# Sandy4321/dist-svgd

Hardware: AMD Instinct MI355X
Metric: SVGD particle-updates/sec (n=65536,d=256) at 1/2/4/8 GPUs + % MFMA/HBM roofline (higher is better)
Workload: dtype f32; 1 GPU; dist-logreg DistSampler all_scores, Jacobi, median bandwidth; n=65536, d=256, N_global=16384, parallelism=dp1, particles_per_gpu=65536

## Files before the change

### dist-svgd_amd/csrc/gemm_x3.hpp

```cpp
#pragma once
#include "gemm_tiles.hpp"

namespace dsvgd {

typedef __bf16 bf16x8 __attribute__((ext_vector_type(8)));
typedef __bf16 bf16x4 __attribute__((ext_vector_type(4)));
typedef uint32_t u32x4 __attribute__((ext_vector_type(4)));
typedef uint32_t u32x2 __attribute__((ext_vector_type(2)));

__device__ __forceinline__ f32x16 mfma_bf16(bf16x8 a, bf16x8 b, f32x16 c) {
  return __builtin_amdgcn_mfma_f32_32x32x16_bf16(a, b, c, 0, 0, 0);
}

struct Split3 {
  __bf16 s0, s1, s2;
};
__device__ __forceinline__ Split3 split3(float v) {
  Split3 o;
  o.s0 = (__bf16)v;
  float r = v - (float)o.s0;
  o.s1 = (__bf16)r;
  r -= (float)o.s1;
  o.s2 = (__bf16)r;
  return o;
}

constexpr int kX3Parts = 3;
constexpr int kX3Step = 16;

__device__ __forceinline__ float lane_select(uint64_t mask, float a, float b) {
  float d;
  asm("v_cndmask_b32 %0, %1, %2, %3" : "=v"(d) : "v"(b), "v"(a), "s"(mask));
  return d;
}

typedef _Float16 f16x8 __attribute__((ext_vector_type(8)));
typedef _Float16 f16x4 __attribute__((ext_vector_type(4)));

struct FmtX3 {
  using E = __bf16;
  using V8 = bf16x8;
  using V4 = bf16x4;
  static constexpr int P = 3;
  static constexpr float kAScale = 1.f;
  static constexpr float kAScaleLog2 = 0.f;
};
struct FmtH2 {
  using E = _Float16;
  using V8 = f16x8;
  using V4 = f16x4;
  static constexpr int P = 2;
  static constexpr float kAScale = 32768.f;
  static constexpr float kAScaleLog2 = 15.f;
};

template <class F>
__device__ __forceinline__ f32x16 mfma_fmt(typename F::V8 a, typename F::V8 b, f32x16 c) {
  if constexpr (F::P == 3)
    return __builtin_amdgcn_mfma_f32_32x32x16_bf16(a, b, c, 0, 0, 0);
  else
    return __builtin_amdgcn_mfma_f32_32x32x16_f16(a, b, c, 0, 0, 0);
}

template <class F>
__device__ __forceinline__ void split_fmt(float v, typename F::E (&o)[F::P]) {
  if constexpr (F::P == 3) {
    const Split3 s = split3(v);
    o[0] = s.s0;
    o[1] = s.s1;
    o[2] = s.s2;
  } else {
    o[0] = (_Float16)v;
    o[1] = (_Float16)(v - (float)o[0]);
  }
}

template <class F, int TM>
__device__ __forceinline__ void mfma_products(const typename F::V8 (&a)[TM][F::P],
                                              const typename F::V8 (&b)[F::P], f32x16* acc) {
  if constexpr (F::P == 3) {
#pragma unroll
    for (int mi = 0; mi < TM; ++mi) acc[mi] = mfma_fmt<F>(a[mi][2], b[0], acc[mi]);
#pragma unroll
    for (int mi = 0; mi < TM; ++mi) acc[mi] = mfma_fmt<F>(a[mi][1], b[1], acc[mi]);
#pragma unroll
    for (int mi = 0; mi < TM; ++mi) acc[mi] = mfma_fmt<F>(a[mi][0], b[2], acc[mi]);
  }
#pragma unroll
  for (int mi = 0; mi < TM; ++mi) acc[mi] = mfma_fmt<F>(a[mi][1], b[0], acc[mi]);
#pragma unroll
  for (int mi = 0; mi < TM; ++mi) acc[mi] = mfma_fmt<F>(a[mi][0], b[1], acc[mi]);
#pragma unroll
  for (int mi = 0; mi < TM; ++mi) acc[mi] = mfma_fmt<F>(a[mi][0], b[0], acc[mi]);
}

__device__ __forceinline__ int x3_off(int x, int h) { return x * 32 + ((h ^ ((x >> 3) & 1)) << 4); }

template <int TN, bool DMA = true, bool EXP = true, bool M16 = false, int RW = 2, class F = FmtX3,
          int NB = 2, int FAM = kFamRBF>
struct NNX3Tile {
  static constexpr int P = F::P;
  static_assert(NB == 2 || (NB == 3 && DMA), "3-stage ring: DMA path");
  static constexpr int ND = NB;
  using V8 = typename F::V8;
  static_assert(!M16 || P == 3, "the 16x16x32 concatenated-k form is the 3-part format's");
  static constexpr int kThreads = 512;
  static constexpr int TM = 2;
  static constexpr int kCW = 8 / RW;
  static constexpr int BM = 64 * RW;
  static constexpr int AR = BM / 128;
  static constexpr int BC = kCW * 32 * TN;
  static_assert(RW == 2 || (RW == 4 && DMA && !EXP), "256-row blocks: DMA path, no exp");
  static constexpr int BJ = kX3Step;
  static constexpr int SA = P * BM * 32;
  static constexpr int SB = P * BC * 32;
  static constexpr int kStage = SA + SB;
  static constexpr int kSmemBytes = NB * kStage + (DMA ? ND * AR * kPanelElems * 4 : 0);
  static constexpr int kBChunks = SB / 16;
  static constexpr int LB = (kBChunks + kThreads - 1) / kThreads;
  static constexpr int kHalf = TN > 1 ? TN / 2 : 1;
  static_assert(kSmemBytes <= 160 * 1024, "LDS budget");
  static_assert(!DMA || kBChunks % kThreads == 0, "DMA: every wave issues LB DMAs");

  f32x16 acc[TM][TN];
  f32x4 acc16[4][2 * TN];
  bf16x8 a16[4][3];
  f32x4 ra;
  int64_t prow = 0;
  u32x4 rb[DMA ? 1 : LB];
  float rs;
  float pw;
  V8 a[TM][P];

  __device__ __forceinline__ float kval(float v, float scale) const {
    if constexpr (FAM == kFamIMQ)
      return imq_pow(v, scale, pw, F::kAScaleLog2);
    else
      return __builtin_amdgcn_exp2f(fmaf(v, scale, F::kAScaleLog2));
  }

  __device__ __forceinline__ void load(const float* __restrict__ Apanels, const typename F::E* __restrict__ Yx,
                                       int64_t ldy, int64_t j0) {
    const int t = threadIdx.x;
    const __amdgpu_buffer_rsrc_t rA =
        __builtin_amdgcn_make_buffer_rsrc((void*)Apanels, (short)0, 0x7fffffff, 0x00020000);
    const __amdgpu_buffer_rsrc_t rB =
        __builtin_amdgcn_make_buffer_rsrc((void*)Yx, (short)0, 0x7fffffff, 0x00020000);
    const int soA = (int)((j0 >> 4) * kPanelElems * 4);
    const int soB = (int)((j0 >> 4) * P * ldy * 32);
    ra = __builtin_bit_cast(f32x4, __builtin_amdgcn_raw_buffer_load_b128(rA, t * 16, soA, 0));
#pragma unroll
    for (int u = 0; u < LB; ++u) {
      const int f = t + u * kThreads;
      if (kBChunks % kThreads == 0 || f < kBChunks) {
        const int p = f / (2 * BC), rem = f % (2 * BC);
        rb[u] = __builtin_bit_cast(
            u32x4, __builtin_amdgcn_raw_buffer_load_b128(rB, (int)(p * ldy * 32 + rem * 16), soB, 0));
      }
    }
  }

  __device__ __forceinline__ void store(char* st, float scale, int64_t dgl) {
    store_a(st, scale, dgl);
    const int t = threadIdx.x;
#pragma unroll
    for (int u = 0; u < LB; ++u) {
      const int f = t + u * kThreads;
      if (kBChunks % kThreads == 0 || f < kBChunks)
        *reinterpret_cast<u32x4*>(st + SA + f * 16) = rb[u];
    }
  }

  __device__ __forceinline__ void store_a(char* st, float scale, int64_t dgl, int a = 0) {
    const int t = threadIdx.x, row = (t >> 2) + 128 * a, c4 = t & 3;
    if (!EXP) {
      if constexpr (F::kAScale != 1.f) {
#pragma unroll
        for (int q = 0; q < 4; ++q) ra[q] *= F::kAScale;
      }
    } else if (dgl > -BM && dgl < BJ) {
      const int qd = (int)dgl + row - 4 * c4;
#pragma unroll
      for (int q = 0; q < 4; ++q)
        ra[q] = (qd == q) ? 0.f : kval(ra[q], scale);
    } else {
#pragma unroll
      for (int q = 0; q < 4; ++q) ra[q] = kval(ra[q], scale);
    }
    if (EXP) rs += (ra[0] + ra[1]) + (ra[2] + ra[3]);
    typename F::V4 sp[P];
#pragma unroll
    for (int q = 0; q < 4; ++q) {
      typename F::E v[P];
      split_fmt<F>(ra[q], v);
#pragma unroll
      for (int p = 0; p < P; ++p) sp[p][q] = v[p];
    }
    const int off = (M16 ? row * 32 + ((c4 >> 1) << 4) : x3_off(row, c4 >> 1)) + ((c4 & 1) << 3);
#pragma unroll
    for (int p = 0; p < P; ++p) *reinterpret_cast<typename F::V4*>(st + p * BM * 32 + off) = sp[p];
  }

  static constexpr int kRaw = NB * kStage;
  static constexpr int kSlot = AR * kPanelElems * 4;
  static constexpr int kDAux = 2;

  template <int AUX = 0>
  __device__ __forceinline__ static void dma16(__amdgpu_buffer_rsrc_t r, char* lds, int voff,
                                               int soff) {
    __builtin_amdgcn_raw_ptr_buffer_load_lds(r, (__attribute__((address_space(3))) void*)lds, 16,
                                             voff, soff, 0, AUX);
  }

  __device__ __forceinline__ void dma_b(char* st, __amdgpu_buffer_rsrc_t rB, int64_t ldy,
                                        int64_t j0) {
    const int t = threadIdx.x, wbase = __builtin_amdgcn_readfirstlane(t >> 6) * 64;
    const int soB = (int)((j0 >> 4) * P * ldy * 32);
#pragma unroll
    for (int u = 0; u < LB; ++u) {
      const int f = t + u * kThreads, p = f / (2 * BC), rem = f % (2 * BC);
      dma16(rB, st + SA + (wbase + u * kThreads) * 16, (int)(p * ldy * 32 + rem * 16), soB);
    }
  }

  __device__ __forceinline__ void dma_d(char* raw, __amdgpu_buffer_rsrc_t rA, int64_t j0) {
    const int t = threadIdx.x;
    if (transposed(j0)) {
      const float* src = sym_D + (((j0 >> 7) * sym_pcols + sym_I * 8) * kPanelElems +
                                   (j0 & 127) * 16);
      const __amdgpu_buffer_rsrc_t rT =
          __builtin_amdgcn_make_buffer_rsrc((void*)src, (short)0, 0x7fffffff, 0x00020000);
      dma16<kDAux>(rT, raw + __builtin_amdgcn_readfirstlane(t >> 6) * 1024, (t >> 6) * kPanelElems * 4 + (t & 63) * 16, 0);
      return;
    }
#pragma unroll
    for (int a = 0; a < AR; ++a)
      dma16<kDAux>(rA, raw + a * kPanelElems * 4 + __builtin_amdgcn_readfirstlane(t >> 6) * 1024, (int)(a * prow) + t * 16,
                   (int)((j0 >> 4) * kPanelElems * 4));
  }

  __device__ __forceinline__ f32x4 raw_read(const char* raw, int64_t j0, int a = 0) const {
    const int t = threadIdx.x;
    if (RW == 2 && transposed(j0)) {
      const int row = t >> 2, c4 = t & 3;
      const float* r = reinterpret_cast<const float*>(raw) + (row >> 4) * 256 + (row & 15) +
                       (4 * c4) * 16;
      float v[4];
#pragma unroll
      for (int e = 0; e < 4; ++e) v[e] = r[((e + c4) & 3) * 16];
      constexpr uint64_t kOdd = 0xAAAAAAAAAAAAAAAAull, kHi2 = 0xCCCCCCCCCCCCCCCCull;
      float w[4];
#pragma unroll
      for (int q = 0; q < 4; ++q) w[q] = lane_select(kOdd, v[(q + 3) & 3], v[q]);
#pragma unroll
      for (int q = 0; q < 4; ++q) v[q] = lane_select(kHi2, w[(q + 2) & 3], w[q]);
      return f32x4{v[0], v[1], v[2], v[3]};
    }
    return *reinterpret_cast<const f32x4*>(raw + a * kPanelElems * 4 + t * 16);
  }

  int64_t kst = BJ;
  const float* sym_D = nullptr;
  int64_t sym_pcols = 0;
  int64_t sym_I = 0;
  __device__ __forceinline__ bool transposed(int64_t j0) const {
    return sym_D != nullptr && (j0 >> 7) < sym_I;
  }

  __device__ __forceinline__ void read_a(const char* st, int wr) {
    if (M16) {
      const int lane = threadIdx.x & 63, rr = lane & 15, g = lane >> 4, hh = g & 1;
#pragma unroll
      for (int mt = 0; mt < 4; ++mt) {
        const int off = (wr * 64 + mt * 16 + rr) * 32 + hh * 16;
        const int sl = g >> 1;
        a16[mt][0] = *reinterpret_cast<const bf16x8*>(st + sl * BM * 32 + off);
        a16[mt][1] = *reinterpret_cast<const bf16x8*>(st + (sl ^ 1) * BM * 32 + off);
        a16[mt][2] = *reinterpret_cast<const bf16x8*>(st + 2 * sl * BM * 32 + off);
      }
      return;
    }
    const int lane = threadIdx.x & 63, r = lane & 31, h = lane >> 5;
#pragma unroll
    for (int mi = 0; mi < TM; ++mi)
#pragma unroll
      for (int p = 0; p < P; ++p)
        a[mi][p] = *reinterpret_cast<const V8*>(st + p * BM * 32 +
                                                x3_off(wr * 32 * TM + mi * 32 + r, h));
  }

  template <int N0, int N1>
  __device__ __forceinline__ void compute(const char* st, int wc) {
    if (M16) {
      const int lane = threadIdx.x & 63, rr = lane & 15, g = lane >> 4, hh = g & 1;
      const int s = g >> 1;
#pragma unroll
      for (int nt = 2 * N0; nt < 2 * N1; ++nt) {
        const char* bb = st + SA + (wc * 32 * TN + nt * 16 + rr) * 32 + hh * 16;
        const bf16x8 g1 = *reinterpret_cast<const bf16x8*>(bb + s * BC * 32);
        const bf16x8 g3 = *reinterpret_cast<const bf16x8*>(bb + (2 - 2 * s) * BC * 32);
#pragma unroll
        for (int mt = 0; mt < 4; ++mt)
          acc16[mt][nt] = __builtin_amdgcn_mfma_f32_16x16x32_bf16(a16[mt][2], g3, acc16[mt][nt], 0, 0, 0);
#pragma unroll
        for (int mt = 0; mt < 4; ++mt)
          acc16[mt][nt] = __builtin_amdgcn_mfma_f32_16x16x32_bf16(a16[mt][1], g1, acc16[mt][nt], 0, 0, 0);
#pragma unroll
        for (int mt = 0; mt < 4; ++mt)
          acc16[mt][nt] = __builtin_amdgcn_mfma_f32_16x16x32_bf16(a16[mt][0], g1, acc16[mt][nt], 0, 0, 0);
      }
      return;
    }
    const int lane = threadIdx.x & 63, r = lane & 31, h = lane >> 5;
#pragma unroll
    for (int ni = N0; ni < N1; ++ni) {
      V8 b[P];
#pragma unroll
      for (int p = 0; p < P; ++p)
        b[p] = *reinterpret_cast<const V8*>(st + SA + p * BC * 32 +
                                            x3_off(wc * 32 * TN + ni * 32 + r, h));
      f32x16 c[TM];
#pragma unroll
      for (int mi = 0; mi < TM; ++mi) c[mi] = acc[mi][ni];
      mfma_products<F, TM>(a, b, c);
#pragma unroll
      for (int mi = 0; mi < TM; ++mi) acc[mi][ni] = c[mi];
    }
  }

  __device__ __forceinline__ static void lds_barrier() {
    asm volatile("s_waitcnt lgkmcnt(0)\n\ts_barrier" ::: "memory");
  }

  __device__ __forceinline__ void run(const float* __restrict__ Apanels, const typename F::E* __restrict__ Yx,
                                      int64_t ldy, int64_t k0, int64_t k1, float scale, char* smem,
                                      int64_t row_g0) {
    const int w = __builtin_amdgcn_readfirstlane((int)(threadIdx.x >> 6)), wr = w / kCW, wc = w % kCW;
    rs = 0.f;
#pragma unroll
    for (int mi = 0; mi < TM; ++mi)
#pragma unroll
      for (int ni = 0; ni < TN; ++ni)
#pragma unroll
        for (int q = 0; q < 16; ++q) acc[mi][ni][q] = 0.f;
#pragma unroll
    for (int mt = 0; mt < 4; ++mt)
#pragma unroll
      for (int nt = 0; nt < 2 * TN; ++nt) acc16[mt][nt] = f32x4{0.f, 0.f, 0.f, 0.f};
    if (k0 >= k1) return;
    if (DMA) {
      const __amdgpu_buffer_rsrc_t rA =
          __builtin_amdgcn_make_buffer_rsrc((void*)Apanels, (short)0, 0x7fffffff, 0x00020000);
      const __amdgpu_buffer_rsrc_t rB =
          __builtin_amdgcn_make_buffer_rsrc((void*)Yx, (short)0, 0x7fffffff, 0x00020000);
      char* raw = smem + kRaw;
      if constexpr (NB == 3) {
        dma_b(smem, rB, ldy, k0);
        dma_d(raw, rA, k0);
        if (k0 + kst < k1) {
          dma_b(smem + kStage, rB, ldy, k0 + kst);
          dma_d(raw + kSlot, rA, k0 + kst);
          asm volatile("s_waitcnt vmcnt(%0)" ::"n"(LB + AR) : "memory");
        } else {
          asm volatile("s_waitcnt vmcnt(0)" ::: "memory");
        }
#pragma unroll
        for (int a = 0; a < AR; ++a) {
          ra = raw_read(raw, k0, a);
          store_a(smem, scale, row_g0 - k0, a);
        }
        asm volatile("s_waitcnt lgkmcnt(0)\n\ts_barrier" ::: "memory");
        for (int64_t j0 = k0; j0 < k1; j0 += 3 * kst) {
          step_dma3<0>(rA, rB, ldy, j0, k1, scale, smem, row_g0, wr, wc);
          if (j0 + kst < k1) step_dma3<1>(rA, rB, ldy, j0 + kst, k1, scale, smem, row_g0, wr, wc);
          if (j0 + 2 * kst < k1)
            step_dma3<2>(rA, rB, ldy, j0 + 2 * kst, k1, scale, smem, row_g0, wr, wc);
        }
// ... 318 lines not shown
```

### dist-svgd_amd/csrc/phi_w1.hpp

```cpp
#pragma once
#include "gemm_x3.hpp"

namespace dsvgd {

struct PhiW1 {
  static constexpr int kThreads = 256;
  static constexpr int BM = 128, BC = 512, BJ = 16, P = 2;
  static constexpr int SA = P * BM * 32;
  static constexpr int kSmemBytes = 2 * SA;
  static constexpr int kScrLd = 44;
  static constexpr int kScrBytes = 16 * kScrLd * 4;
};

constexpr int kW1Sgb = 4;
__device__ __forceinline__ f32x4 w1_load(__amdgpu_buffer_rsrc_t r, int voff, int soff) {
  return __builtin_bit_cast(f32x4, __builtin_amdgcn_raw_buffer_load_b128(r, voff, soff, 0));
}
__device__ __forceinline__ f32x4 w1_load_nt(__amdgpu_buffer_rsrc_t r, int voff, int soff) {
  return __builtin_bit_cast(f32x4, __builtin_amdgcn_raw_buffer_load_b128(r, voff, soff, 2));
}

constexpr int w1_waves(int NI, bool EXP) { return NI == 2 && EXP ? 2 : 1; }
template <int DS, int NI = 4, bool EXP = true, int FAM = kFamRBF, class... PW>
__global__ __launch_bounds__(256)
__attribute__((amdgpu_waves_per_eu(w1_waves(NI, EXP), w1_waves(NI, EXP)))) void phi_w1_kernel(
    const float* A, int64_t a_npad, const _Float16* Yx, int64_t ldy,
    int64_t K, int64_t kchunk, const dsvgd_select_state* __restrict__ st, float* __restrict__ C,
    int64_t ldc, float* __restrict__ rowsum, int64_t m, int64_t row0, int sym,
    const float* __restrict__ colinv, int slice0, const float* __restrict__ gate, int gate_on,
    int ks_begin = 0, int ks_wrap = 0, int tcol0 = 0, int t_per = 0, int t_first = 0,
    int t_nblk = 1, int64_t t_ostride = 0, PW... pw_) {
  static_assert(sizeof...(PW) == (FAM == kFamIMQ ? 1 : 0), "pw: the IMQ instantiations only");
  [[maybe_unused]] const float pw = (0.f + ... + pw_);
  static_assert(NI == 4 || NI == 2, "NI: 4 or 2 column tiles per wave");
  static_assert(EXP || DS == 0, "the identity form is DS 0 only");
  const bool want_rs = EXP || rowsum != nullptr;
  if (gate && ((*gate != 0.f) != (gate_on != 0))) return;
  using F = FmtH2;
  constexpr int BC = 4 * 32 * NI;
  using V8 = F::V8;
  constexpr int P = PhiW1::P;
  constexpr bool TRK = DS == 1 || DS == 3 || DS == 4;
  __shared__ __attribute__((aligned(16))) char smem[PhiW1::kSmemBytes + (TRK ? 4 * PhiW1::kScrBytes : 0)];
  const int t = threadIdx.x, lane = t & 63, r = lane & 31, h = lane >> 5;
  const int w = __builtin_amdgcn_readfirstlane(t >> 6);
  const int64_t lin = (int64_t)blockIdx.z * gridDim.y + blockIdx.y;
  const bool xm = ((DS == 4 || DS == 0) && t_per == 1) || (DS == 3 && t_per > 0 && tcol0 == 1);
  const int64_t lid = lin * gridDim.x + blockIdx.x;
  const int64_t xu = (lid >> 3) * (8 / gridDim.z) + (lid & 7) / gridDim.z;
  const int64_t cbx = xm ? xu % gridDim.x : blockIdx.x;
  const int64_t by = xm ? xu / gridDim.x
                   : DS == 2 ? lin / gridDim.z
                   : DS == 1 ? (int64_t)gridDim.y - 1 - lin / gridDim.z : blockIdx.y;
  const int64_t bz = xm ? (lid & 7) % gridDim.z
                   : (DS == 1 || DS == 2) ? lin % gridDim.z : blockIdx.z;
  const bool tb = DS == 3 && t_per > 0;
  const int64_t tpart = tb ? by / t_per : 0;
  const int64_t byl = tb ? by % t_per : by;
  const int64_t i0 = byl * PhiW1::BM;
  const int64_t c0 = cbx * BC + w * 32 * NI;
  const int64_t kb0 = bz * kchunk, kend = min(K, kb0 + kchunk);
  int ks0 = (int)(kb0 / PhiW1::BJ) + (DS == 0 ? ks_begin : 0);
  int nsteps = kend > kb0 ? (int)((kend - kb0) / PhiW1::BJ) : 0;
  const int Z = (int)gridDim.z;
  const int kdir = DS == 2 ? -Z : DS == 1 ? Z : 1;
  auto wrapk = [&](int ks) { return (DS == 0 && ks_wrap > 0 && ks >= ks_wrap) ? ks - ks_wrap : ks; };
  const int kyoff = DS == 3 ? ks_begin : 0;
  if (DS == 2) {
    const int T = (int)((K - i0) / PhiW1::BJ);
    ks0 = (int)(K / PhiW1::BJ) - 1 - (int)bz;
    nsteps = T > bz ? (T - (int)bz + Z - 1) / Z : 0;
  } else if (DS == 1) {
    const int T = (int)(i0 / PhiW1::BJ);
    ks0 = (int)bz;
    nsteps = T > bz ? (T - (int)bz + Z - 1) / Z : 0;
  }
  const int ksp = DS == 4 ? (int)min(max(kb0, i0), kend) / PhiW1::BJ : 0;
  if (tb) {
    const int64_t at = ((int64_t)bz * (gridDim.y / t_per) + tpart) * t_ostride;
    C += at;
    rowsum += at;
  } else {
    C += (int64_t)(slice0 + bz) * m * ldc;
    rowsum += (int64_t)(slice0 + bz) * roundup128(m);
  }
  const float scale = !EXP ? 0.f : FAM == kFamIMQ ? st->inv_h : -st->inv_h * kLog2e;

  const __amdgpu_buffer_rsrc_t rD = __builtin_amdgcn_make_buffer_rsrc(
      (void*)(A + (i0 >> 7) * (a_npad >> 4) * kPanelElems), (short)0, 0x7fffffff, 0x00020000);
  const __amdgpu_buffer_rsrc_t rB =
      __builtin_amdgcn_make_buffer_rsrc((void*)(Yx + c0 * 16), (short)0, 0x7fffffff, 0x00020000);
  const int pstride = (int)(ldy * 32);
  const int vB = x3_off(r, h);
  const int vD = t * 32;
  const int srow = t >> 1, shalf = t & 1;
  const int aoff = x3_off(srow, shalf);
  auto diag0 = [&](int kfirst) {
    int64_t dg = row0 + i0 + srow - 8 * shalf - (int64_t)kfirst * PhiW1::BJ;
    if (DS == 0 && ks_wrap > 0 && row0 + i0 + srow < (int64_t)ks_begin * PhiW1::BJ)
      dg += (int64_t)ks_wrap * PhiW1::BJ;
    return (int)max(min(dg, (int64_t)(1 << 30)), (int64_t)-(1 << 30));
  };

  f32x16 acc[4][NI];
#pragma unroll
  for (int mi = 0; mi < 4; ++mi)
#pragma unroll
    for (int ni = 0; ni < NI; ++ni)
#pragma unroll
      for (int q = 0; q < 16; ++q) acc[mi][ni][q] = 0.f;
  float rs = 0.f;

  const int symI = tb ? (int)(((t_first + tpart) % t_nblk) * t_per + byl)
                   : DS == 3 ? tcol0 + (int)by : (sym || DS == 4) ? (int)(i0 >> 7) : -1;
  const int64_t pcols = a_npad >> 4;
  const int vP = (t >> 5) * kPanelElems * 4 + (t & 31) * 32;
  float* const scr = reinterpret_cast<float*>(smem + PhiW1::kSmemBytes + w * PhiW1::kScrBytes);
  const int sw_off = ((lane & 31) >> 1) * PhiW1::kScrLd + 16 * (lane >> 5) + 8 * (lane & 1);
  const int sr_off = 8 * shalf * PhiW1::kScrLd + (lane >> 1);

  auto phase = [&](auto TR_, const int ks0, const int nsteps, const int qd0) {
    constexpr bool TR = decltype(TR_)::value;
    if (nsteps <= 0) return;
    V8 b[NI][P];
    f32x4 dr[4][2];
    f32x4 tr[2];
    const int last = nsteps - 1;
    auto loadB = [&](int ni, int k) {
      const int soff = (wrapk(ks0 + kdir * min(k, last)) + kyoff) * P * pstride;
#pragma unroll
      for (int p = 0; p < P; ++p)
        b[ni][p] = __builtin_bit_cast(V8, w1_load(rB, vB + ni * 1024, soff + p * pstride));
    };
    auto loadD = [&](f32x4 (&d)[2], int k) {
      const int kc = min(k, last);
      const int64_t j0 = (int64_t)wrapk(ks0 + kdir * kc) * PhiW1::BJ;
      if constexpr (TR) {
        const float* src = A + (((j0 >> 7) * pcols + symI * 8) * kPanelElems + (j0 & 127) * 16);
        const __amdgpu_buffer_rsrc_t rT =
            __builtin_amdgcn_make_buffer_rsrc((void*)src, (short)0, 0x7fffffff, 0x00020000);
        d[0] = w1_load_nt(rT, vP, 0);
        d[1] = w1_load_nt(rT, vP + 16, 0);
      } else {
        const int soff = (int)(j0 >> 4) * kPanelElems * 4;
        d[0] = w1_load_nt(rD, vD, soff);
        d[1] = w1_load_nt(rD, vD + 16, soff);
      }
    };
    auto transpose = [&](const f32x4 (&d)[2], f32x4 (&o)[2]) {
      *reinterpret_cast<f32x4*>(scr + sw_off) = d[0];
      *reinterpret_cast<f32x4*>(scr + sw_off + 4) = d[1];
#pragma unroll
      for (int q = 0; q < 8; ++q) o[q >> 2][q & 3] = scr[sr_off + q * PhiW1::kScrLd];
    };
    auto stage = [&](char* st_, const f32x4 (&d)[2], int k) {
      const int qd = max(min(qd0 - kdir * k * PhiW1::BJ, 8), -1);
      float e[8];
#pragma unroll
      for (int q = 0; q < 8; ++q) {
        const float v = q < 4 ? d[0][q] : d[1][q - 4];
        const float x = !EXP ? v * F::kAScale
                        : FAM == kFamIMQ ? imq_pow(v, scale, pw, F::kAScaleLog2)
                                         : __builtin_amdgcn_exp2f(fmaf(v, scale, F::kAScaleLog2));
        e[q] = (EXP && !TR && qd == q) ? 0.f : x;
      }
      const float s = ((e[0] + e[1]) + (e[2] + e[3])) + ((e[4] + e[5]) + (e[6] + e[7]));
      rs += k <= last ? s : 0.f;
      V8 p0, p1;
#pragma unroll
      for (int q = 0; q < 8; ++q) {
        const _Float16 a0 = (_Float16)e[q];
        p0[q] = a0;
        p1[q] = (_Float16)(e[q] - (float)a0);
      }
      *reinterpret_cast<V8*>(st_ + aoff) = p0;
      *reinterpret_cast<V8*>(st_ + PhiW1::BM * 32 + aoff) = p1;
    };
    auto barrier = []() { asm volatile("s_waitcnt lgkmcnt(0)\n\ts_barrier" ::: "memory"); };
    auto step = [&](int k, const char* cur, char* nxt, const f32x4 (&ds_)[2], f32x4 (&dl)[2],
                    const f32x4 (&dt)[2]) {
      V8 a[4][P];
#pragma unroll
      for (int mi = 0; mi < 4; ++mi)
#pragma unroll
        for (int p = 0; p < P; ++p)
          a[mi][p] = *reinterpret_cast<const V8*>(cur + p * PhiW1::BM * 32 + x3_off(mi * 32 + r, h));
      if constexpr (TR)
        stage(nxt, tr, k + 1);
      else
        stage(nxt, ds_, k + 1);
#pragma unroll
      for (int ni = 0; ni < NI; ++ni) {
#pragma unroll
        for (int mi = 0; mi < 4; ++mi) acc[mi][ni] = mfma_fmt<F>(a[mi][1], b[ni][0], acc[mi][ni]);
#pragma unroll
        for (int mi = 0; mi < 4; ++mi) acc[mi][ni] = mfma_fmt<F>(a[mi][0], b[ni][1], acc[mi][ni]);
#pragma unroll
        for (int mi = 0; mi < 4; ++mi) acc[mi][ni] = mfma_fmt<F>(a[mi][0], b[ni][0], acc[mi][ni]);
        loadB(ni, k + 1);
      }
      if constexpr (TR) transpose(dt, tr);
      __builtin_amdgcn_sched_group_barrier(0x100, 8, 0);
#pragma unroll
      for (int i = 0; i < 4 * NI; ++i) {
        __builtin_amdgcn_sched_group_barrier(0x008, 1, 0);
        __builtin_amdgcn_sched_group_barrier(0x002, kW1Sgb, 0);
      }
      __builtin_amdgcn_sched_group_barrier(0x200, 2, 0);
#pragma unroll
      for (int i = 0; i < 8 * NI; ++i) {
        __builtin_amdgcn_sched_group_barrier(0x008, 1, 0);
        if (TR && i == 1) __builtin_amdgcn_sched_group_barrier(0x200, 2, 0);
        if (TR && i >= 2 && i < 10) __builtin_amdgcn_sched_group_barrier(0x100, 1, 0);
        if (i % 4 == 3) __builtin_amdgcn_sched_group_barrier(0x020, 1, 0);
      }
      loadD(dl, k + 3);
    };

#pragma unroll
    for (int ni = 0; ni < NI; ++ni) loadB(ni, 0);
    loadD(dr[0], 0);
    loadD(dr[1], 1);
    loadD(dr[2], 2);
    if constexpr (TR) {
      transpose(dr[0], tr);
      stage(smem, tr, 0);
      transpose(dr[1], tr);
    } else {
      stage(smem, dr[0], 0);
    }
    barrier();
    for (int k = 0; k < nsteps; k += 8) {
      step(k, smem, smem + PhiW1::SA, dr[1], dr[3], dr[2]);
      barrier();
      if (k + 1 >= nsteps) break;
      step(k + 1, smem + PhiW1::SA, smem, dr[2], dr[0], dr[3]);
      barrier();
      if (k + 2 >= nsteps) break;
      step(k + 2, smem, smem + PhiW1::SA, dr[3], dr[1], dr[0]);
      barrier();
      if (k + 3 >= nsteps) break;
      step(k + 3, smem + PhiW1::SA, smem, dr[0], dr[2], dr[1]);
      barrier();
      if (k + 4 >= nsteps) break;
      step(k + 4, smem, smem + PhiW1::SA, dr[1], dr[3], dr[2]);
      barrier();
      if (k + 5 >= nsteps) break;
      step(k + 5, smem + PhiW1::SA, smem, dr[2], dr[0], dr[3]);
      barrier();
      if (k + 6 >= nsteps) break;
      step(k + 6, smem, smem + PhiW1::SA, dr[3], dr[1], dr[0]);
      barrier();
      if (k + 7 >= nsteps) break;
      step(k + 7, smem + PhiW1::SA, smem, dr[0], dr[2], dr[1]);
      barrier();
    }
  };
  if constexpr (DS == 4) {
    phase(std::true_type{}, ks0, ksp - ks0, 0);
    phase(std::false_type{}, ksp, ks0 + nsteps - ksp, diag0(ksp));
  } else {
    phase(std::integral_constant<bool, DS == 1 || DS == 3>{}, ks0, nsteps, diag0(ks0));
  }

#pragma unroll
  for (int mi = 0; mi < 4; ++mi)
#pragma unroll
    for (int ni = 0; ni < NI; ++ni) {
      const int64_t col = c0 + ni * 32 + r;
      const float cs = colinv[col] * (1.f / F::kAScale);
#pragma unroll
      for (int q = 0; q < 16; ++q) {
        const int64_t row = i0 + mi * 32 + c_row(q, lane);
        if (row < m) C[row * ldc + col] = acc[mi][ni][q] * cs;
      }
    }
  {
    const float v = rs + __shfl_xor(rs, 1, 64);
    if (want_rs && cbx == 0 && shalf == 0 && i0 + srow < m)
      rowsum[i0 + srow] = v * (1.f / F::kAScale);
  }
}

}
```

### dist-svgd_amd/csrc/phi_w2.hpp

```cpp
#pragma once
#include "phi_w1.hpp"

namespace dsvgd {

struct PhiW2 {
  static constexpr int kThreads = 256;
  static constexpr int BM = 256, BC = 256, BJ = 16, P = 2;
  static constexpr int SA = P * BM * 32;
  static constexpr int kSmemBytes = 2 * SA;
};

#ifndef DSVGD_W2_SGB
#define DSVGD_W2_SGB 6
#endif
#ifndef DSVGD_W2_MF
#define DSVGD_W2_MF 40
#endif
constexpr int kW2Sgb = DSVGD_W2_SGB, kW2Mf = DSVGD_W2_MF;

template <int DS>
__global__ __launch_bounds__(256) __attribute__((amdgpu_waves_per_eu(1, 1))) void phi_w2_kernel(
    const float* A, int64_t a_npad, int64_t a_rows, const _Float16* Wh, int64_t ldw, int64_t K,
    int64_t kchunk, const dsvgd_select_state* __restrict__ st, float* __restrict__ C, int64_t ldc,
    float* __restrict__ rowsum, int64_t m, int64_t row0, const float* __restrict__ colinv,
    const float* __restrict__ gate, int xm) {
  static_assert(DS == 0 || DS == 4, "DS: 0 (full layout) or 4 (symmetric, one launch)");
  if (gate && *gate != 0.f) return;
  using F = FmtH2;
  using V8 = F::V8;
  constexpr int P = PhiW2::P, BM = PhiW2::BM;
  constexpr bool SYM = DS == 4;
  __shared__ __attribute__((aligned(16))) char smem[PhiW2::kSmemBytes + (SYM ? 8 * PhiW1::kScrBytes : 0)];
  const int t = threadIdx.x, lane = t & 63, r = lane & 31, h = lane >> 5;
  const int w = __builtin_amdgcn_readfirstlane(t >> 6);
  const int wr = w >> 1, wc = w & 1;
  const int64_t lid = ((int64_t)blockIdx.z * gridDim.y + blockIdx.y) * gridDim.x + blockIdx.x;
  const int64_t xu = (lid >> 3) * (8 / gridDim.z) + (lid & 7) / gridDim.z;
  const int64_t cbx = xm ? xu % gridDim.x : blockIdx.x;
  const int64_t by = xm ? xu / gridDim.x : blockIdx.y;
  const int64_t bz = xm ? (lid & 7) % gridDim.z : blockIdx.z;
  const int64_t i0 = by * BM;
  const int64_t c0 = cbx * PhiW2::BC + wc * 128;
  const int64_t kb0 = bz * kchunk, kend = min(K, kb0 + kchunk);
  const int ks0 = (int)(kb0 / PhiW2::BJ);
  const int nsteps = kend > kb0 ? (int)((kend - kb0) / PhiW2::BJ) : 0;
  C += bz * m * ldc;
  rowsum += bz * roundup128(m);
  const float scale = -st->inv_h * kLog2e;
  const bool live1 = i0 + 128 < a_rows;
  const int64_t pcols = a_npad >> 4;
  const __amdgpu_buffer_rsrc_t rD0 = __builtin_amdgcn_make_buffer_rsrc(
      (void*)(A + (i0 >> 7) * pcols * kPanelElems), (short)0, 0x7fffffff, 0x00020000);
  const __amdgpu_buffer_rsrc_t rD1 = __builtin_amdgcn_make_buffer_rsrc(
      (void*)(A + ((i0 >> 7) + (live1 ? 1 : 0)) * pcols * kPanelElems), (short)0,
      live1 ? 0x7fffffff : 0, 0x00020000);
  const __amdgpu_buffer_rsrc_t rB =
      __builtin_amdgcn_make_buffer_rsrc((void*)(Wh + c0 * 16), (short)0, 0x7fffffff, 0x00020000);
  const int pstride = (int)(ldw * 32);
  const int vB = x3_off(r, h);
  const int vD = t * 32;
  const int srow = t >> 1, shalf = t & 1;
  const int aoff = x3_off(srow, shalf);
  auto diag0 = [&](int kfirst, int hb) {
    const int64_t dg = row0 + i0 + 128 * hb + srow - 8 * shalf - (int64_t)kfirst * PhiW2::BJ;
    return (int)max(min(dg, (int64_t)(1 << 30)), (int64_t)-(1 << 30));
  };

  f32x16 acc[4][4];
#pragma unroll
  for (int mi = 0; mi < 4; ++mi)
#pragma unroll
    for (int ni = 0; ni < 4; ++ni)
#pragma unroll
      for (int q = 0; q < 16; ++q) acc[mi][ni][q] = 0.f;
  float rs0 = 0.f, rs1 = 0.f;

  const int symI = (int)(i0 >> 7);
  const int vP = (t >> 5) * kPanelElems * 4 + (t & 31) * 32;
  float* const scr0 = reinterpret_cast<float*>(smem + PhiW2::kSmemBytes + w * PhiW1::kScrBytes);
  float* const scr1 = scr0 + 4 * (PhiW1::kScrBytes / 4);
  const int sw_off = ((lane & 31) >> 1) * PhiW1::kScrLd + 16 * (lane >> 5) + 8 * (lane & 1);
  const int sr_off = 8 * shalf * PhiW1::kScrLd + (lane >> 1);

  auto phase = [&](auto TR0_, auto TR1_, const int ks0, const int nsteps, const int qd0,
                   const int qd1) {
    constexpr bool TR0 = decltype(TR0_)::value, TR1 = decltype(TR1_)::value;
    if (nsteps <= 0) return;
    V8 b[4][P];
    f32x4 dr[4][2][2];
    f32x4 tr[2][2];
    const int last = nsteps - 1;
    auto loadB = [&](int ni, int k) {
      const int soff = (ks0 + min(k, last)) * P * pstride;
#pragma unroll
      for (int p = 0; p < P; ++p)
        b[ni][p] = __builtin_bit_cast(V8, w1_load(rB, vB + ni * 1024, soff + p * pstride));
    };
    auto loadD = [&](f32x4 (&d)[2][2], int k) {
      const int64_t j0 = (int64_t)(ks0 + min(k, last)) * PhiW2::BJ;
      const int soff = (int)(j0 >> 4) * kPanelElems * 4;
      auto one = [&](auto TR_, int hb, f32x4 (&o)[2]) {
        if constexpr (decltype(TR_)::value) {
          const bool ok = hb == 0 || live1;
          const float* src = A + (((j0 >> 7) * pcols + (symI + (ok ? hb : 0)) * 8) * kPanelElems +
                                  (j0 & 127) * 16);
          const __amdgpu_buffer_rsrc_t rT = __builtin_amdgcn_make_buffer_rsrc(
              (void*)src, (short)0, ok ? 0x7fffffff : 0, 0x00020000);
          o[0] = w1_load_nt(rT, vP, 0);
          o[1] = w1_load_nt(rT, vP + 16, 0);
        } else {
          o[0] = w1_load_nt(hb ? rD1 : rD0, vD, soff);
          o[1] = w1_load_nt(hb ? rD1 : rD0, vD + 16, soff);
        }
      };
      one(TR0_, 0, d[0]);
      one(TR1_, 1, d[1]);
    };
    auto transpose = [&](float* scr, const f32x4 (&d)[2], f32x4 (&o)[2]) {
      *reinterpret_cast<f32x4*>(scr + sw_off) = d[0];
      *reinterpret_cast<f32x4*>(scr + sw_off + 4) = d[1];
#pragma unroll
      for (int q = 0; q < 8; ++q) o[q >> 2][q & 3] = scr[sr_off + q * PhiW1::kScrLd];
    };
    auto stage = [&](char* st_, const f32x4 (&d)[2], int k, bool tr_, int qd0_, float& rs) {
      const int qd = max(min(qd0_ - k * PhiW2::BJ, 8), -1);
      float e[8];
#pragma unroll
      for (int q = 0; q < 8; ++q) {
        const float v = q < 4 ? d[0][q] : d[1][q - 4];
        const float x = __builtin_amdgcn_exp2f(fmaf(v, scale, F::kAScaleLog2));
        e[q] = (!tr_ && qd == q) ? 0.f : x;
      }
      const float s = ((e[0] + e[1]) + (e[2] + e[3])) + ((e[4] + e[5]) + (e[6] + e[7]));
      rs += k <= last ? s : 0.f;
      V8 p0, p1;
#pragma unroll
      for (int q = 0; q < 8; ++q) {
        const _Float16 a0 = (_Float16)e[q];
        p0[q] = a0;
        p1[q] = (_Float16)(e[q] - (float)a0);
      }
      *reinterpret_cast<V8*>(st_ + aoff) = p0;
      *reinterpret_cast<V8*>(st_ + BM * 32 + aoff) = p1;
    };
    auto stage2 = [&](char* st_, const f32x4 (&d)[2][2], int k) {
      if constexpr (TR0) stage(st_, tr[0], k, true, qd0, rs0);
      else stage(st_, d[0], k, false, qd0, rs0);
      if constexpr (TR1) stage(st_ + 128 * 32, tr[1], k, true, qd1, rs1);
      else stage(st_ + 128 * 32, d[1], k, false, qd1, rs1);
    };
    auto barrier = []() { asm volatile("s_waitcnt lgkmcnt(0)\n\ts_barrier" ::: "memory"); };
    auto step = [&](int k, const char* cur, char* nxt, const f32x4 (&ds_)[2][2],
                    f32x4 (&dl)[2][2], const f32x4 (&dt)[2][2]) {
      V8 a[4][P];
#pragma unroll
      for (int mi = 0; mi < 4; ++mi)
#pragma unroll
        for (int p = 0; p < P; ++p)
          a[mi][p] = *reinterpret_cast<const V8*>(cur + p * BM * 32 +
                                                  x3_off(wr * 128 + mi * 32 + r, h));
      stage2(nxt, ds_, k + 1);
#pragma unroll
      for (int ni = 0; ni < 4; ++ni) {
#pragma unroll
        for (int mi = 0; mi < 4; ++mi) acc[mi][ni] = mfma_fmt<F>(a[mi][1], b[ni][0], acc[mi][ni]);
#pragma unroll
        for (int mi = 0; mi < 4; ++mi) acc[mi][ni] = mfma_fmt<F>(a[mi][0], b[ni][1], acc[mi][ni]);
#pragma unroll
        for (int mi = 0; mi < 4; ++mi) acc[mi][ni] = mfma_fmt<F>(a[mi][0], b[ni][0], acc[mi][ni]);
        loadB(ni, k + 1);
      }
      if constexpr (TR0) transpose(scr0, dt[0], tr[0]);
      if constexpr (TR1) transpose(scr1, dt[1], tr[1]);
      __builtin_amdgcn_sched_group_barrier(0x100, 8, 0);
#pragma unroll
      for (int i = 0; i < kW2Mf; ++i) {
        __builtin_amdgcn_sched_group_barrier(0x008, 1, 0);
        __builtin_amdgcn_sched_group_barrier(0x002, kW2Sgb, 0);
        if (i % 12 == 11) __builtin_amdgcn_sched_group_barrier(0x020, 2, 0);
      }
      __builtin_amdgcn_sched_group_barrier(0x200, 4, 0);
#pragma unroll
      for (int i = kW2Mf; i < 48; ++i) {
        __builtin_amdgcn_sched_group_barrier(0x008, 1, 0);
        if (i % 12 == 11) __builtin_amdgcn_sched_group_barrier(0x020, 2, 0);
      }
      loadD(dl, k + 3);
    };

#pragma unroll
    for (int ni = 0; ni < 4; ++ni) loadB(ni, 0);
    loadD(dr[0], 0);
    loadD(dr[1], 1);
    loadD(dr[2], 2);
    if constexpr (TR0) transpose(scr0, dr[0][0], tr[0]);
    if constexpr (TR1) transpose(scr1, dr[0][1], tr[1]);
    stage2(smem, dr[0], 0);
    if constexpr (TR0) transpose(scr0, dr[1][0], tr[0]);
    if constexpr (TR1) transpose(scr1, dr[1][1], tr[1]);
    barrier();
    for (int k = 0; k < nsteps; k += 4) {
      step(k, smem, smem + PhiW2::SA, dr[1], dr[3], dr[2]);
      barrier();
      if (k + 1 >= nsteps) break;
      step(k + 1, smem + PhiW2::SA, smem, dr[2], dr[0], dr[3]);
      barrier();
      if (k + 2 >= nsteps) break;
      step(k + 2, smem, smem + PhiW2::SA, dr[3], dr[1], dr[0]);
      barrier();
      if (k + 3 >= nsteps) break;
      step(k + 3, smem + PhiW2::SA, smem, dr[0], dr[2], dr[1]);
      barrier();
    }
  };
  using T_ = std::true_type;
  using F_ = std::false_type;
  if constexpr (SYM) {
    const int kse = ks0 + nsteps;
    const int ka = min(max(ks0, (int)(i0 >> 4)), kse), kb = min(max(ks0, (int)(i0 >> 4) + 8), kse);
    phase(T_{}, T_{}, ks0, ka - ks0, 0, 0);
    phase(F_{}, T_{}, ka, kb - ka, diag0(ka, 0), 0);
    phase(F_{}, F_{}, kb, kse - kb, diag0(kb, 0), diag0(kb, 1));
  } else {
    phase(F_{}, F_{}, ks0, nsteps, diag0(ks0, 0), diag0(ks0, 1));
  }

#pragma unroll
  for (int mi = 0; mi < 4; ++mi)
#pragma unroll
    for (int ni = 0; ni < 4; ++ni) {
      const int64_t col = c0 + ni * 32 + r;
      const float cs = colinv[col] * (1.f / F::kAScale);
#pragma unroll
      for (int q = 0; q < 16; ++q) {
        const int64_t row = i0 + wr * 128 + mi * 32 + c_row(q, lane);
        if (row < m) C[row * ldc + col] = acc[mi][ni][q] * cs;
      }
    }
  {
    const float v0 = rs0 + __shfl_xor(rs0, 1, 64), v1 = rs1 + __shfl_xor(rs1, 1, 64);
    if (cbx == 0 && shalf == 0) {
      if (i0 + srow < m) rowsum[i0 + srow] = v0 * (1.f / F::kAScale);
      if (i0 + 128 + srow < m) rowsum[i0 + 128 + srow] = v1 * (1.f / F::kAScale);
    }
  }
}

}
```

Before: 4.924 million particle-updates/s.

## Use packed fma_mix f16 split, peel diagonal masking, and retune W1 schedule groups

Replaces the per-element f32→f16 hi/lo split with packed conversions plus v_fma_mixlo/mixhi residual computation in both phi kernels, cutting VALU instructions in the staging path. In phi_w1 the diagonal-zeroing select is peeled out: a wave-uniform ballot checks whether an 8-step block can touch the diagonal and runs a mask-free body otherwise. The row-sum reduction gets asm barriers to fix its association order, and the sched_group_barrier interleave for the NI=2 variant is made tunable and retuned. These changes add inline asm and more code paths, which raises the risk of scheduling or register-pressure regressions.

New measurement: 4.960 million particle-updates/s (median of 6 runs). Within noise of the previous version (+0.7%).

```diff
diff --git a/dist-svgd_amd/csrc/gemm_x3.hpp b/dist-svgd_amd/csrc/gemm_x3.hpp
--- a/dist-svgd_amd/csrc/gemm_x3.hpp
+++ b/dist-svgd_amd/csrc/gemm_x3.hpp
@@ -73,6 +73,28 @@
     o[0] = (_Float16)v;
     o[1] = (_Float16)(v - (float)o[0]);
   }
+}
+
+typedef _Float16 f16x2 __attribute__((ext_vector_type(2)));
+__device__ __forceinline__ void split_h2_pair(float e0, float e1, uint32_t& hi, uint32_t& lo) {
+  const f16x2 h = {(_Float16)e0, (_Float16)e1};
+  hi = __builtin_bit_cast(uint32_t, h);
+  asm("v_fma_mixlo_f16 %0, %1, -1.0, %2 op_sel_hi:[1,0,0]" : "=v"(lo) : "v"(hi), "v"(e0));
+  asm("v_fma_mixhi_f16 %0, %1, -1.0, %2 op_sel:[1,0,0] op_sel_hi:[1,0,0]"
+      : "+v"(lo)
+      : "v"(hi), "v"(e1));
+}
+__device__ __forceinline__ void split_h2_x8(const float (&e)[8], f16x8& p0, f16x8& p1) {
+  u32x4 hi, lo;
+#pragma unroll
+  for (int q = 0; q < 4; ++q) {
+    uint32_t a, b;
+    split_h2_pair(e[2 * q], e[2 * q + 1], a, b);
+    hi[q] = a;
+    lo[q] = b;
+  }
+  p0 = __builtin_bit_cast(f16x8, hi);
+  p1 = __builtin_bit_cast(f16x8, lo);
 }
 
 template <class F, int TM>
diff --git a/dist-svgd_amd/csrc/phi_w1.hpp b/dist-svgd_amd/csrc/phi_w1.hpp
--- a/dist-svgd_amd/csrc/phi_w1.hpp
+++ b/dist-svgd_amd/csrc/phi_w1.hpp
@@ -12,12 +12,43 @@
   static constexpr int kScrBytes = 16 * kScrLd * 4;
 };
 
-constexpr int kW1Sgb = 4;
+#ifndef DSVGD_W1_SGB
+#define DSVGD_W1_SGB 5
+#endif
+#ifndef DSVGD_W1_GAPS
+#define DSVGD_W1_GAPS 8
+#endif
+#ifndef DSVGD_W1_TRANS
+#define DSVGD_W1_TRANS 0
+#endif
+constexpr int w1_sgb(int NI) { return NI == 2 ? DSVGD_W1_SGB : 4; }
+constexpr int w1_gaps(int NI) { return NI == 2 ? DSVGD_W1_GAPS : 4 * NI; }
+constexpr bool w1_sgb_trans(int NI) { return NI == 2 && DSVGD_W1_TRANS != 0; }
+#ifndef DSVGD_W1_SPLIT
+#define DSVGD_W1_SPLIT 1
+#endif
+#ifndef DSVGD_W1_PEEL
+#define DSVGD_W1_PEEL 1
+#endif
+constexpr bool kW1Split = DSVGD_W1_SPLIT != 0, kW1Peel = DSVGD_W1_PEEL != 0;
 __device__ __forceinline__ f32x4 w1_load(__amdgpu_buffer_rsrc_t r, int voff, int soff) {
   return __builtin_bit_cast(f32x4, __builtin_amdgcn_raw_buffer_load_b128(r, voff, soff, 0));
 }
 __device__ __forceinline__ f32x4 w1_load_nt(__amdgpu_buffer_rsrc_t r, int voff, int soff) {
   return __builtin_bit_cast(f32x4, __builtin_amdgcn_raw_buffer_load_b128(r, voff, soff, 2));
+}
+
+__device__ __forceinline__ float w1_sum8(const float (&e)[8]) {
+  float s[4];
+#pragma unroll
+  for (int q = 0; q < 4; ++q) {
+    s[q] = e[2 * q] + e[2 * q + 1];
+    asm("" : "+v"(s[q]));
+  }
+  float a = s[0] + s[1], b = s[2] + s[3];
+  asm("" : "+v"(a));
+  asm("" : "+v"(b));
+  return a + b;
 }
 
 constexpr int w1_waves(int NI, bool EXP) { return NI == 2 && EXP ? 2 : 1; }
@@ -121,6 +152,8 @@
 
   auto phase = [&](auto TR_, const int ks0, const int nsteps, const int qd0) {
     constexpr bool TR = decltype(TR_)::value;
+    constexpr std::true_type yes{};
+    [[maybe_unused]] constexpr std::false_type no{};
     if (nsteps <= 0) return;
     V8 b[NI][P];
     f32x4 dr[4][2];
@@ -153,8 +186,9 @@
 #pragma unroll
       for (int q = 0; q < 8; ++q) o[q >> 2][q & 3] = scr[sr_off + q * PhiW1::kScrLd];
     };
-    auto stage = [&](char* st_, const f32x4 (&d)[2], int k) {
-      const int qd = max(min(qd0 - kdir * k * PhiW1::BJ, 8), -1);
+    auto stage = [&](auto DG_, char* st_, const f32x4 (&d)[2], int k) __attribute__((always_inline)) {
+      constexpr bool DG = decltype(DG_)::value && EXP && !TR;
+      [[maybe_unused]] const int qd = max(min(qd0 - kdir * k * PhiW1::BJ, 8), -1);
       float e[8];
 #pragma unroll
       for (int q = 0; q < 8; ++q) {
@@ -162,23 +196,30 @@
         const float x = !EXP ? v * F::kAScale
                         : FAM == kFamIMQ ? imq_pow(v, scale, pw, F::kAScaleLog2)
                                          : __builtin_amdgcn_exp2f(fmaf(v, scale, F::kAScaleLog2));
-        e[q] = (EXP && !TR && qd == q) ? 0.f : x;
-      }
-      const float s = ((e[0] + e[1]) + (e[2] + e[3])) + ((e[4] + e[5]) + (e[6] + e[7]));
+        if constexpr (DG)
+          e[q] = qd == q ? 0.f : x;
+        else
+          e[q] = x;
+      }
+      const float s = w1_sum8(e);
       rs += k <= last ? s : 0.f;
       V8 p0, p1;
-#pragma unroll
-      for (int q = 0; q < 8; ++q) {
-        const _Float16 a0 = (_Float16)e[q];
-        p0[q] = a0;
-        p1[q] = (_Float16)(e[q] - (float)a0);
+      if constexpr (kW1Split) {
+        split_h2_x8(e, p0, p1);
+      } else {
+#pragma unroll
+        for (int q = 0; q < 8; ++q) {
+          const _Float16 a0 = (_Float16)e[q];
+          p0[q] = a0;
+          p1[q] = (_Float16)(e[q] - (float)a0);
+        }
       }
       *reinterpret_cast<V8*>(st_ + aoff) = p0;
       *reinterpret_cast<V8*>(st_ + PhiW1::BM * 32 + aoff) = p1;
     };
     auto barrier = []() { asm volatile("s_waitcnt lgkmcnt(0)\n\ts_barrier" ::: "memory"); };
-    auto step = [&](int k, const char* cur, char* nxt, const f32x4 (&ds_)[2], f32x4 (&dl)[2],
-                    const f32x4 (&dt)[2]) {
+    auto step = [&](auto DG_, int k, const char* cur, char* nxt, const f32x4 (&ds_)[2],
+                    f32x4 (&dl)[2], const f32x4 (&dt)[2]) __attribute__((always_inline)) {
       V8 a[4][P];
 #pragma unroll
       for (int mi = 0; mi < 4; ++mi)
@@ -186,9 +227,9 @@
         for (int p = 0; p < P; ++p)
           a[mi][p] = *reinterpret_cast<const V8*>(cur + p * PhiW1::BM * 32 + x3_off(mi * 32 + r, h));
       if constexpr (TR)
-        stage(nxt, tr, k + 1);
+        stage(DG_, nxt, tr, k + 1);
       else
-        stage(nxt, ds_, k + 1);
+        stage(DG_, nxt, ds_, k + 1);
 #pragma unroll
       for (int ni = 0; ni < NI; ++ni) {
 #pragma unroll
@@ -200,19 +241,19 @@
         loadB(ni, k + 1);
       }
       if constexpr (TR) transpose(dt, tr);
+      constexpr int kGaps = w1_gaps(NI), kSgb = w1_sgb(NI);
+      constexpr bool kSgbT = w1_sgb_trans(NI);
       __builtin_amdgcn_sched_group_barrier(0x100, 8, 0);
 #pragma unroll
-      for (int i = 0; i < 4 * NI; ++i) {
+      for (int j = 0; j < 12 * NI; ++j) {
+        const int i = j - 4 * NI;
         __builtin_amdgcn_sched_group_barrier(0x008, 1, 0);
-        __builtin_amdgcn_sched_group_barrier(0x002, kW1Sgb, 0);
-      }
-      __builtin_amdgcn_sched_group_barrier(0x200, 2, 0);
-#pragma unroll
-      for (int i = 0; i < 8 * NI; ++i) {
-        __builtin_amdgcn_sched_group_barrier(0x008, 1, 0);
+        if (j < kGaps) __builtin_amdgcn_sched_group_barrier(0x002, kSgb, 0);
+        if (j < kGaps && j < 8 && kSgbT) __builtin_amdgcn_sched_group_barrier(0x400, 1, 0);
+        if (j == kGaps - 1) __builtin_amdgcn_sched_group_barrier(0x200, 2, 0);
         if (TR && i == 1) __builtin_amdgcn_sched_group_barrier(0x200, 2, 0);
         if (TR && i >= 2 && i < 10) __builtin_amdgcn_sched_group_barrier(0x100, 1, 0);
-        if (i % 4 == 3) __builtin_amdgcn_sched_group_barrier(0x020, 1, 0);
+        if (i >= 0 && i % 4 == 3) __builtin_amdgcn_sched_group_barrier(0x020, 1, 0);
       }
       loadD(dl, k + 3);
     };
@@ -224,37 +265,55 @@
     loadD(dr[2], 2);
     if constexpr (TR) {
       transpose(dr[0], tr);
-      stage(smem, tr, 0);
+      stage(yes, smem, tr, 0);
       transpose(dr[1], tr);
     } else {
-      stage(smem, dr[0], 0);
+      stage(yes, smem, dr[0], 0);
     }
     barrier();
-    for (int k = 0; k < nsteps; k += 8) {
-      step(k, smem, smem + PhiW1::SA, dr[1], dr[3], dr[2]);
-      barrier();
-      if (k + 1 >= nsteps) break;
-      step(k + 1, smem + PhiW1::SA, smem, dr[2], dr[0], dr[3]);
-      barrier();
-      if (k + 2 >= nsteps) break;
-      step(k + 2, smem, smem + PhiW1::SA, dr[3], dr[1], dr[0]);
-      barrier();
-      if (k + 3 >= nsteps) break;
-      step(k + 3, smem + PhiW1::SA, smem, dr[0], dr[2], dr[1]);
-      barrier();
-      if (k + 4 >= nsteps) break;
-      step(k + 4, smem, smem + PhiW1::SA, dr[1], dr[3], dr[2]);
-      barrier();
-      if (k + 5 >= nsteps) break;
-      step(k + 5, smem + PhiW1::SA, smem, dr[2], dr[0], dr[3]);
-      barrier();
-      if (k + 6 >= nsteps) break;
-      step(k + 6, smem, smem + PhiW1::SA, dr[3], dr[1], dr[0]);
-      barrier();
-      if (k + 7 >= nsteps) break;
-      step(k + 7, smem + PhiW1::SA, smem, dr[0], dr[2], dr[1]);
-      barrier();
+#define DSVGD_W1_BODY(DG_, LEAVE)                                     \
+  step(DG_, k, smem, smem + PhiW1::SA, dr[1], dr[3], dr[2]);          \
+  barrier();                                                          \
+  if (k + 1 >= nsteps) LEAVE;                                         \
+  step(DG_, k + 1, smem + PhiW1::SA, smem, dr[2], dr[0], dr[3]);      \
+  barrier();                                                          \
+  if (k + 2 >= nsteps) LEAVE;                                         \
+  step(DG_, k + 2, smem, smem + PhiW1::SA, dr[3], dr[1], dr[0]);      \
+  barrier();                                                          \
+  if (k + 3 >= nsteps) LEAVE;                                         \
+  step(DG_, k + 3, smem + PhiW1::SA, smem, dr[0], dr[2], dr[1]);      \
+  barrier();                                                          \
+  if (k + 4 >= nsteps) LEAVE;                                         \
+  step(DG_, k + 4, smem, smem + PhiW1::SA, dr[1], dr[3], dr[2]);      \
+  barrier();                                                          \
+  if (k + 5 >= nsteps) LEAVE;                                         \
+  step(DG_, k + 5, smem + PhiW1::SA, smem, dr[2], dr[0], dr[3]);      \
+  barrier();                                                          \
+  if (k + 6 >= nsteps) LEAVE;                                         \
+  step(DG_, k + 6, smem, smem + PhiW1::SA, dr[3], dr[1], dr[0]);      \
+  barrier();                                                          \
+  if (k + 7 >= nsteps) LEAVE;                                         \
+  step(DG_, k + 7, smem + PhiW1::SA, smem, dr[0], dr[2], dr[1]);      \
+  barrier();
+    if constexpr (EXP && !TR && kW1Peel) {
+      auto near = [&](int k) {
+        const int64_t qa = qd0 - (int64_t)kdir * PhiW1::BJ * (k + 1);
+        const int64_t qb = qd0 - (int64_t)kdir * PhiW1::BJ * (k + 8);
+        return __builtin_amdgcn_ballot_w64(max(qa, qb) >= 0 && min(qa, qb) <= 7) != 0;
+      };
+      for (int k = 0; k < nsteps; k += 8) {
+        for (; k < nsteps && !near(k); k += 8) {
+          DSVGD_W1_BODY(no, { k = nsteps; break; })
+        }
+        if (k >= nsteps) break;
+        DSVGD_W1_BODY(yes, break)
+      }
+    } else {
+      for (int k = 0; k < nsteps; k += 8) {
+        DSVGD_W1_BODY(yes, break)
+      }
     }
+#undef DSVGD_W1_BODY
   };
   if constexpr (DS == 4) {
     phase(std::true_type{}, ks0, ksp - ks0, 0);
diff --git a/dist-svgd_amd/csrc/phi_w2.hpp b/dist-svgd_amd/csrc/phi_w2.hpp
--- a/dist-svgd_amd/csrc/phi_w2.hpp
+++ b/dist-svgd_amd/csrc/phi_w2.hpp
@@ -134,12 +134,7 @@
       const float s = ((e[0] + e[1]) + (e[2] + e[3])) + ((e[4] + e[5]) + (e[6] + e[7]));
       rs += k <= last ? s : 0.f;
       V8 p0, p1;
-#pragma unroll
-      for (int q = 0; q < 8; ++q) {
-        const _Float16 a0 = (_Float16)e[q];
-        p0[q] = a0;
-        p1[q] = (_Float16)(e[q] - (float)a0);
-      }
+      split_h2_x8(e, p0, p1);
       *reinterpret_cast<V8*>(st_ + aoff) = p0;
       *reinterpret_cast<V8*>(st_ + BM * 32 + aoff) = p1;
     };
```
